# fundamentalvision/BEVFormer

Measured on AMD Instinct MI355X. Metric: BEV-encoder queries/sec (200x200 BEV, 6 cams, 4 lvls), higher is better.
Workload: dtype f32/bf16x3; 1 GPU; bevformer_base BEV encoder forward, 1 frame/step, 200x200 queries, 6 cams, 4 levels, 6 layers, with history BEV; sca_row_order=image, global_batch=1, parallelism=single GPU

## Files before the change

### bevformer_amd/csrc/bevmsda_linear.hip

```cpp
#include "../../include/bevmsda.h"
#include "linear_mfma.h"
#include "linear_pipe.h"
#include "linear_panel.h"
#include "linear_roles.h"
#include "linear_chain.h"
#include "wgrad_mfma.h"
#include "wgrad_tr.h"

namespace {
constexpr bool kLinearPipeDefault = false;
constexpr long long kLinearPipeMaxRows = 8192;
constexpr long long kChainSmallRows = 8192;
inline bool misaligned(const void *p) { return (reinterpret_cast<uintptr_t>(p) & 15u) != 0; }
}

extern "C" {

static int linear_launch(const float *x0, const float *a0, const float *x1, const float *a1, const float *w,
                         const uint16_t *wpack, const float *bias, const bevmsda_linear_desc *d, float *y,
                         void *stream, const int32_t *gidx = nullptr, const float *gscale = nullptr,
                         const float *mask = nullptr, long ldmask = 0, float mask_scale = 1.0f) {
  if (!d) return BEVMSDA_ERR_NULL_POINTER;
  if (d->M < 0 || d->N < 0 || d->K0 < 0 || d->K1 < 0) return BEVMSDA_ERR_BAD_SHAPE;
  if (d->precision != 0 && d->precision != 1) return BEVMSDA_ERR_BAD_OPTION;
// ... 166 lines not shown
  if (nprob < 0 || nprob > bevmsda::kWgMaxProblems || M < 0) return BEVMSDA_ERR_BAD_SHAPE;
  if (precision != 0 && precision != 1) return BEVMSDA_ERR_BAD_OPTION;
  if (nprob == 0 || M == 0) return BEVMSDA_OK;
  if (!probs) return BEVMSDA_ERR_NULL_POINTER;
  if (variant == 2 && workgroups == 0) {
    long long t2 = 0;
    for (int i = 0; i < nprob; ++i) t2 += 1LL * ((probs[i].N + 255) / 256) * ((probs[i].K + 127) / 128);
    const long long s2 = t2 > 0 ? (256 / t2 / 8) * 8 : 0;
    if (s2 < 8 || t2 * s2 < 208) variant = 0;
  }
  bevmsda::WgradMultiArgs a{};
  long long tiles = 0;
  for (int i = 0; i < nprob; ++i) {
    const bevmsda_wgrad_problem &q = probs[i];
    if (q.N <= 0 || q.K <= 0) return BEVMSDA_ERR_BAD_SHAPE;
    if (q.N % 4 != 0 || q.K % 4 != 0 || q.ldg % 4 != 0 || q.ldx % 4 != 0) return BEVMSDA_ERR_UNSUPPORTED;
    if (q.ldg < q.N || q.ldx < q.K || q.ldgw < q.K) return BEVMSDA_ERR_BAD_SHAPE;
    if (!q.g || !q.x || !q.grad_w) return BEVMSDA_ERR_NULL_POINTER;
    if (misaligned(q.g) || misaligned(q.x) || (reinterpret_cast<uintptr_t>(q.grad_w) & 3u) != 0) return BEVMSDA_ERR_MISALIGNED;
    bevmsda::WgradArgs &w = a.p[i];
    w.g = q.g; w.x = q.x; w.ldg = q.ldg; w.ldx = q.ldx; w.gw = q.grad_w; w.ldgw = q.ldgw; w.gb = q.grad_b; w.M = M;
    w.N = q.N; w.K = q.K; w.tiles_n = (q.N + (variant == 2 ? 255 : 127)) / (variant == 2 ? 256 : 128); w.tiles_k = (q.K + 127) / 128;
    a.tile0[i] = static_cast<int>(tiles);
    tiles += 1LL * w.tiles_n * w.tiles_k;
  }
  if (tiles >= (1LL << 20)) return BEVMSDA_ERR_TOO_LARGE;
  a.tile0[nprob] = static_cast<int>(tiles);
  a.nprob = nprob;
  if (workgroups < 0 || workgroups > (1 << 20)) return BEVMSDA_ERR_BAD_OPTION;
  long long slices = workgroups > 0 ? workgroups / tiles : (tiles >= 12 ? (768 + tiles - 1) / tiles : 512 / tiles);
  if (variant == 2 && workgroups == 0) {
    slices = (256 / tiles / 8) * 8;
    if (slices < 8) slices = 8;
  }
  if (slices < 1) slices = 1;
  long long rows = (M + slices - 1) / slices;
  rows = ((rows + 31) / 32) * 32;
  if (rows < 128) rows = 128;
  slices = (M + rows - 1) / rows;
  for (int i = 0; i < nprob; ++i) a.p[i].rows_per_block = static_cast<int>(rows);
  const long long slices8 = ((slices + 7) / 8) * 8;
  if (tiles * slices8 >= (1LL << 31)) return BEVMSDA_ERR_TOO_LARGE;
  const dim3 grid(static_cast<unsigned>(tiles * slices8)), block(256);
  hipStream_t st = static_cast<hipStream_t>(stream);
  if (variant == 2) {
    if (precision == 0) hipLaunchKernelGGL((bevmsda::wgrad_tr2_multi_kernel<3>), grid, dim3(512), 0, st, a);
    else hipLaunchKernelGGL((bevmsda::wgrad_tr2_multi_kernel<1>), grid, dim3(512), 0, st, a);
  } else if (variant == 0) {
    if (precision == 0) hipLaunchKernelGGL((bevmsda::wgrad_tr_multi_kernel<3>), grid, block, 0, st, a);
    else hipLaunchKernelGGL((bevmsda::wgrad_tr_multi_kernel<1>), grid, block, 0, st, a);
  } else {
    if (precision == 0) hipLaunchKernelGGL((bevmsda::wgrad_multi_kernel<3>), grid, block, 0, st, a);
    else hipLaunchKernelGGL((bevmsda::wgrad_multi_kernel<1>), grid, block, 0, st, a);
  }
  return hipGetLastError() == hipSuccess ? BEVMSDA_OK : BEVMSDA_ERR_LAUNCH;
}

int64_t bevmsda_linear_packed_bytes(int N, int K) {
  if (N <= 0 || K <= 0 || K % 32 != 0) return 0;
  return static_cast<int64_t>((N + 127) / 128) * (K / 32) * 2 * 128 * 40 * 2;
}

int bevmsda_linear_pack_weight_f32(const float *w, int64_t ldw, int N, int K, uint16_t *blob, void *stream) {
  if (N <= 0 || K <= 0) return BEVMSDA_ERR_BAD_SHAPE;
  if (K % 32 != 0 || ldw % 4 != 0) return BEVMSDA_ERR_UNSUPPORTED;
  if (ldw < K) return BEVMSDA_ERR_BAD_SHAPE;
  if (!w || !blob) return BEVMSDA_ERR_NULL_POINTER;
  if (misaligned(w) || misaligned(blob)) return BEVMSDA_ERR_MISALIGNED;
  const long long threads = static_cast<long long>((N + 127) / 128) * 128 * (K / 8);
  const long long nb = (threads + 255) / 256;
  if (nb >= (1LL << 31)) return BEVMSDA_ERR_TOO_LARGE;
  hipLaunchKernelGGL(bevmsda::lin_pack_weight_kernel<false>, dim3(static_cast<unsigned>(nb)), dim3(256), 0,
                     static_cast<hipStream_t>(stream), w, static_cast<long>(ldw), N, K, blob);
  return hipGetLastError() == hipSuccess ? BEVMSDA_OK : BEVMSDA_ERR_LAUNCH;
}

int bevmsda_linear_pack_weight_t_f32(const float *wt, int64_t ldwt, int N, int K, uint16_t *blob, void *stream) {
  if (N <= 0 || K <= 0) return BEVMSDA_ERR_BAD_SHAPE;
  if (K % 32 != 0) return BEVMSDA_ERR_UNSUPPORTED;
  if (ldwt < N) return BEVMSDA_ERR_BAD_SHAPE;
  if (!wt || !blob) return BEVMSDA_ERR_NULL_POINTER;
  if (misaligned(blob) || (reinterpret_cast<uintptr_t>(wt) & 3u)) return BEVMSDA_ERR_MISALIGNED;
  const long long threads = static_cast<long long>((N + 127) / 128) * 128 * (K / 8);
  const long long nb = (threads + 255) / 256;
  if (nb >= (1LL << 31)) return BEVMSDA_ERR_TOO_LARGE;
  hipLaunchKernelGGL(bevmsda::lin_pack_weight_kernel<true>, dim3(static_cast<unsigned>(nb)), dim3(256), 0,
                     static_cast<hipStream_t>(stream), wt, static_cast<long>(ldwt), N, K, blob);
  return hipGetLastError() == hipSuccess ? BEVMSDA_OK : BEVMSDA_ERR_LAUNCH;
}

int64_t bevmsda_linear_panel_packed_bytes(int N, int K) {
  if (N <= 0 || K <= 0 || K % bevmsda::kPanelK != 0) return 0;
  return static_cast<int64_t>((N + 63) / 64) * 2 * (K / 16) * 2 * 1024;
}

int bevmsda_linear_panel_pack_weight_f32(const float *w, int64_t ldw, int N, int K, uint16_t *blob, void *stream) {
  if (N <= 0 || K <= 0) return BEVMSDA_ERR_BAD_SHAPE;
  if (K % bevmsda::kPanelK != 0 || ldw % 4 != 0) return BEVMSDA_ERR_UNSUPPORTED;
  if (ldw < K) return BEVMSDA_ERR_BAD_SHAPE;
  if (!w || !blob) return BEVMSDA_ERR_NULL_POINTER;
  if (misaligned(w) || misaligned(blob)) return BEVMSDA_ERR_MISALIGNED;
  const int tiles32 = ((N + 63) / 64) * 2;
  const long long threads = 1LL * tiles32 * (K / 16) * 64;
  const long long nb = (threads + 255) / 256;
  if (nb >= (1LL << 31)) return BEVMSDA_ERR_TOO_LARGE;
  hipLaunchKernelGGL(bevmsda::lin_panel_pack_weight_kernel<false>, dim3(static_cast<unsigned>(nb)), dim3(256), 0,
                     static_cast<hipStream_t>(stream), w, static_cast<long>(ldw), N, K, tiles32, blob);
  return hipGetLastError() == hipSuccess ? BEVMSDA_OK : BEVMSDA_ERR_LAUNCH;
}

int bevmsda_linear_panel_pack_weight_t_f32(const float *wt, int64_t ldwt, int N, int K, uint16_t *blob, void *stream) {
  if (N <= 0 || K <= 0) return BEVMSDA_ERR_BAD_SHAPE;
  if (K % bevmsda::kPanelK != 0) return BEVMSDA_ERR_UNSUPPORTED;
  if (ldwt < N) return BEVMSDA_ERR_BAD_SHAPE;
  if (!wt || !blob) return BEVMSDA_ERR_NULL_POINTER;
  if (misaligned(blob) || (reinterpret_cast<uintptr_t>(wt) & 3u)) return BEVMSDA_ERR_MISALIGNED;
  const int tiles32 = ((N + 63) / 64) * 2;
  const long long threads = 1LL * tiles32 * (K / 16) * 64;
  const long long nb = (threads + 255) / 256;
  if (nb >= (1LL << 31)) return BEVMSDA_ERR_TOO_LARGE;
  hipLaunchKernelGGL(bevmsda::lin_panel_pack_weight_kernel<true>, dim3(static_cast<unsigned>(nb)), dim3(256), 0,
                     static_cast<hipStream_t>(stream), wt, static_cast<long>(ldwt), N, K, tiles32, blob);
  return hipGetLastError() == hipSuccess ? BEVMSDA_OK : BEVMSDA_ERR_LAUNCH;
}

int64_t bevmsda_linear_pack_job_blocks(int N, int K, int kind) {
  if (N <= 0 || K <= 0 || kind < 0 || kind > 3) return 0;
  if (kind & 2) {
    if (K % bevmsda::kPanelK != 0) return 0;
    const long long threads = 1LL * ((N + 63) / 64) * 2 * (K / 16) * 64;
    return (threads + 255) / 256;
  }
  if (K % 32 != 0) return 0;
  const long long threads = static_cast<long long>((N + 127) / 128) * 128 * (K / 8);
  return (threads + 255) / 256;
}

int bevmsda_linear_pack_weights_multi_f32(const bevmsda_pack_job *jobs, int njobs, int64_t blocks, void *stream) {
  static_assert(sizeof(bevmsda_pack_job) == sizeof(bevmsda::PackJob), "bevmsda_pack_job layout");
  if (njobs < 0 || blocks < 0) return BEVMSDA_ERR_BAD_SHAPE;
  if (njobs == 0 || blocks == 0) return BEVMSDA_OK;
  if (!jobs) return BEVMSDA_ERR_NULL_POINTER;
  if (misaligned(jobs)) return BEVMSDA_ERR_MISALIGNED;
  if (blocks >= (1LL << 31)) return BEVMSDA_ERR_TOO_LARGE;
  hipLaunchKernelGGL(bevmsda::lin_pack_weights_multi_kernel, dim3(static_cast<unsigned>(blocks)), dim3(256), 0,
                     static_cast<hipStream_t>(stream), reinterpret_cast<const bevmsda::PackJob *>(jobs), njobs);
  return hipGetLastError() == hipSuccess ? BEVMSDA_OK : BEVMSDA_ERR_LAUNCH;
}

static constexpr int kPanelSkewDefault = 0;
static constexpr long kPanelRolesMinRows = 65536;
static constexpr int kPanelRolesMinCols = 1024;
static constexpr bool kPanelRolesNtStores = true;

static int panel_launch(const float *x0, const float *a0, const float *x1, const float *a1, const int32_t *idx,
                        const float *scale, const uint16_t *wpanel, const float *bias,
                        const bevmsda_linear_desc *d, const bevmsda_layernorm_desc *ln, float *y, void *stream,
                        const int32_t *seg_start, int64_t seg_len, const int64_t *level_shapes, int num_levels,
                        const float *xb = nullptr, int64_t m_split = 0, const int32_t *need = nullptr,
                        int64_t need_rows = 0, int64_t need_len = 0) {
  if (!d) return BEVMSDA_ERR_NULL_POINTER;
  if (d->M < 0 || d->N < 0 || d->K0 < 0 || d->K1 < 0 || d->group_cols < 0) return BEVMSDA_ERR_BAD_SHAPE;
  if (xb && (m_split < 0 || m_split > d->M)) return BEVMSDA_ERR_BAD_SHAPE;
  if (xb && (d->K1 != 0 || a0 || idx || ln || seg_start)) return BEVMSDA_ERR_UNSUPPORTED;
  if (xb && misaligned(xb)) return BEVMSDA_ERR_MISALIGNED;
  if (d->precision != 0 && d->precision != 1) return BEVMSDA_ERR_BAD_OPTION;
  if (d->M == 0 || d->N == 0) return BEVMSDA_OK;
  const int K = d->K0 + d->K1;
  if ((K != 256 && K != 512) || (d->K0 != 256 && d->K0 != 512) || (d->K1 != 0 && d->K1 != 256)) return BEVMSDA_ERR_UNSUPPORTED;
  if (!x0 || !wpanel || !y || (d->K1 > 0 && !x1)) return BEVMSDA_ERR_NULL_POINTER;
  if ((idx == nullptr) != (scale == nullptr)) return BEVMSDA_ERR_NULL_POINTER;
  if (idx && (d->K1 != 0 || a0)) return BEVMSDA_ERR_BAD_SHAPE;
  const int gcols = d->group_cols;
  if (d->N % 4 != 0 || d->ldy % 4 != 0 || d->ldx0 % 4 != 0 || (a0 && d->lda0 % 4 != 0) ||
      (d->K1 > 0 && (d->ldx1 % 4 != 0 || (a1 && d->lda1 % 4 != 0))) || (gcols > 0 && (gcols % 64 != 0 || d->N % gcols != 0)))
    return BEVMSDA_ERR_UNSUPPORTED;
  if (d->ldx0 < d->K0 || d->ldy < (gcols > 0 ? gcols : d->N) || (d->K1 > 0 && d->ldx1 < d->K1)) return BEVMSDA_ERR_BAD_SHAPE;
  if (misaligned(x0) || misaligned(wpanel) || misaligned(y) || (bias && misaligned(bias)) || (a0 && misaligned(a0)) ||
      (d->K1 > 0 && (misaligned(x1) || (a1 && misaligned(a1)))))
    return BEVMSDA_ERR_MISALIGNED;
  const int64_t wbytes = bevmsda_linear_panel_packed_bytes(d->N, K);
  if (wbytes >= (1LL << 31)) return BEVMSDA_ERR_TOO_LARGE;
  if (!ln && 128LL * d->ldy * (d->out_bf16 ? 2 : 4) >= (1LL << 31)) return BEVMSDA_ERR_TOO_LARGE;
  bevmsda::PanelArgs a;
  a.x0 = x0; a.a0 = a0; a.x1 = d->K1 > 0 ? x1 : nullptr; a.a1 = d->K1 > 0 ? a1 : nullptr;
  a.ldx0 = d->ldx0; a.lda0 = d->lda0; a.ldx1 = d->ldx1; a.lda1 = d->lda1;
  a.gidx = idx; a.gscale = scale;
  a.wp = wpanel; a.wp_bytes = static_cast<unsigned>(wbytes);
  a.bias = bias; a.y = y; a.ldy = d->ldy; a.M = d->M; a.N = d->N; a.K0 = d->K0; a.K1 = d->K1;
  a.relu = d->relu ? 1 : 0; a.group_cols = gcols; a.out_bf16 = d->out_bf16 ? 1 : 0;
  a.res = nullptr; a.ldres = 0; a.gamma = a.beta = nullptr; a.eps = 0.f;
  a.xb = xb; a.m_split = m_split;
  a.need = need; a.need_rows = need_rows;
  if (need) {
    if (!xb || d->relu || K != 256) return BEVMSDA_ERR_UNSUPPORTED;
    if (need_rows <= 0 || need_len <= 0) return BEVMSDA_ERR_BAD_SHAPE;
    const int64_t longest = m_split > d->M - m_split ? m_split : d->M - m_split;
    if ((longest + need_rows - 1) / need_rows > need_len) return BEVMSDA_ERR_BAD_SHAPE;
    if ((reinterpret_cast<uintptr_t>(need) & 3u) != 0) return BEVMSDA_ERR_MISALIGNED;
    if (d->reserved[3] != 0) return BEVMSDA_ERR_UNSUPPORTED;
  }
  a.seg_start = seg_start; a.seg_len = seg_len; a.level_shapes = level_shapes; a.num_levels = level_shapes ? num_levels : 0;
  if (seg_start && (seg_len <= 0 || num_levels < 0)) return BEVMSDA_ERR_BAD_SHAPE;
  if (ln) {
    if (d->N != 256 || gcols != 0 || d->relu || d->out_bf16) return BEVMSDA_ERR_UNSUPPORTED;
    if (!ln->gamma || !ln->beta) return BEVMSDA_ERR_NULL_POINTER;
    if (misaligned(ln->gamma) || misaligned(ln->beta) || (ln->res && (misaligned(ln->res) || ln->ldres % 4 != 0 || ln->ldres < d->N)))
      return BEVMSDA_ERR_MISALIGNED;
    a.res = ln->res; a.ldres = ln->ldres; a.gamma = ln->gamma; a.beta = ln->beta; a.eps = ln->eps;
  }
  int shape = d->reserved[2];
  if (shape < 0 || shape > 3) return BEVMSDA_ERR_BAD_OPTION;
  if ((K == 512 || ln) && d->N > 256) return BEVMSDA_ERR_UNSUPPORTED;
  const bool roles_form = !idx && !a.a0 && !a.a1 && !ln && K == 256 && d->N % 32 == 0;
  if (shape == 0 && roles_form && d->N >= kPanelRolesMinCols && d->M >= kPanelRolesMinRows) shape = 3;
  bevmsda_linear_desc d_rule;
  if (shape == 3 && !roles_form) {
    d_rule = *d;
    d_rule.reserved[2] = 0;
    d_rule.reserved[3] = 0;
    d = &d_rule;
    shape = 0;
  }
  if (shape == 3) {
    if (d->reserved[3] < 0 || d->reserved[3] > 4) return BEVMSDA_ERR_BAD_OPTION;
    const int knob = d->reserved[3] == 0 ? (kPanelRolesNtStores ? 2 : 0) : d->reserved[3] & 3;
    const long long nb3 = (d->M + 63) / 64;
    if (nb3 >= (1LL << 31)) return BEVMSDA_ERR_TOO_LARGE;
    a.skew = 0;
    const dim3 g3(static_cast<unsigned>(nb3)), b3(bevmsda::kRolesThreads);
    hipStream_t st3 = static_cast<hipStream_t>(stream);
    if (need) {
      if (d->precision == 0) hipLaunchKernelGGL((bevmsda::linear_roles_kernel<3, kPanelRolesNtStores ? 2 : 0, true, true>), g3, b3, 0, st3, a);
      else hipLaunchKernelGGL((bevmsda::linear_roles_kernel<1, kPanelRolesNtStores ? 2 : 0, true, true>), g3, b3, 0, st3, a);
      return hipGetLastError() == hipSuccess ? BEVMSDA_OK : BEVMSDA_ERR_LAUNCH;
    }
#define BEVMSDA_ROLES(NP_)                                                                                                \
    do {                                                                                                                  \
      switch (knob) {                                                                                                     \
        case 0: hipLaunchKernelGGL((bevmsda::linear_roles_kernel<NP_, 0, true>), g3, b3, 0, st3, a); break;               \
        case 1: hipLaunchKernelGGL((bevmsda::linear_roles_kernel<NP_, 0, false>), g3, b3, 0, st3, a); break;              \
        case 2: hipLaunchKernelGGL((bevmsda::linear_roles_kernel<NP_, 2, true>), g3, b3, 0, st3, a); break;               \
        default: hipLaunchKernelGGL((bevmsda::linear_roles_kernel<NP_, 2, false>), g3, b3, 0, st3, a); break;             \
      }                                                                                                                   \
    } while (0)
    if (d->precision == 0) BEVMSDA_ROLES(3); else BEVMSDA_ROLES(1);
#undef BEVMSDA_ROLES
    return hipGetLastError() == hipSuccess ? BEVMSDA_OK : BEVMSDA_ERR_LAUNCH;
  }
  if (shape == 0) shape = d->N >= 1024 && d->M >= 65536 ? 2 : 1;
  const int bm = shape == 1 ? 64 : 128;
  const long long nb = (d->M + bm - 1) / bm;
  if (nb >= (1LL << 31)) return BEVMSDA_ERR_TOO_LARGE;
  hipStream_t st = static_cast<hipStream_t>(stream);
  const dim3 grid(static_cast<unsigned>(nb));
  int ev = d->reserved[3] >= 32 && d->reserved[3] < 64 ? d->reserved[3] - 32 : -1;
  const bool plain = !idx && !a.a0 && !a.a1 && !ln;
  a.skew = plain && d->reserved[3] == 0 ? kPanelSkewDefault : 0;
  if (d->reserved[3] == 97 || d->reserved[3] == 98) {
  } else if (d->reserved[3] >= 64) {
    if (d->reserved[3] > 98 || !plain) return BEVMSDA_ERR_BAD_OPTION;
    a.skew = d->reserved[3] - 64;
  } else if (ev >= 0) {
    if (ev > 4 || idx || a.a0 || a.a1 || ln) return BEVMSDA_ERR_BAD_OPTION;
  } else if (d->reserved[3] != 0 && d->reserved[3] != 2 && d->reserved[3] != 6) {
    return BEVMSDA_ERR_BAD_OPTION;
  }
  if (need) {
#define BEVMSDA_PANEL_MASKED(NP_)                                                                                              \
    do {                                                                                                                       \
      if (shape == 1) hipLaunchKernelGGL((bevmsda::linear_panel_kernel<NP_, 2, 2, 4, false, 0, 0, 0, false, 2, false, true>), grid, dim3(256), 0, st, a); \
      else hipLaunchKernelGGL((bevmsda::linear_panel_kernel<NP_, 4, 1, 8, false, 0, 0, 0, false, 2, false, true>), grid, dim3(512), 0, st, a);           \
    } while (0)
    if (d->precision == 0) BEVMSDA_PANEL_MASKED(3); else BEVMSDA_PANEL_MASKED(1);
#undef BEVMSDA_PANEL_MASKED
    return hipGetLastError() == hipSuccess ? BEVMSDA_OK : BEVMSDA_ERR_LAUNCH;
  }
  const bool deep = d->reserved[3] == 6;
  if (d->reserved[3] == 97 || d->reserved[3] == 98) {
    if (!plain) return BEVMSDA_ERR_BAD_OPTION;
    const dim3 g128(static_cast<unsigned>((d->M + 127) / 128));
    if (d->precision == 0) {
      if (d->reserved[3] == 97) hipLaunchKernelGGL((bevmsda::linear_panel_kernel<3, 4, 2, 4, false, 0, 0, 0, true, 2>), g128, dim3(256), 0, st, a);
      else hipLaunchKernelGGL((bevmsda::linear_panel_kernel<3, 4, 2, 4, false, 0, 0, 0, true, 4>), g128, dim3(256), 0, st, a);
    } else {
      if (d->reserved[3] == 97) hipLaunchKernelGGL((bevmsda::linear_panel_kernel<1, 4, 2, 4, false, 0, 0, 0, true, 2>), g128, dim3(256), 0, st, a);
      else hipLaunchKernelGGL((bevmsda::linear_panel_kernel<1, 4, 2, 4, false, 0, 0, 0, true, 4>), g128, dim3(256), 0, st, a);
    }
    return hipGetLastError() == hipSuccess ? BEVMSDA_OK : BEVMSDA_ERR_LAUNCH;
  }
  if (ev > 0) {
#define BEVMSDA_PANEL_EV(NP_)                                                                                                  \
    do {                                                                                                                       \
      if (shape == 1) {                                                                                                        \
        if (ev == 1) hipLaunchKernelGGL((bevmsda::linear_panel_kernel<NP_, 2, 2, 4, false, 0, 0, 0, true, 2>), grid, dim3(256), 0, st, a);  \
        else if (ev == 2) hipLaunchKernelGGL((bevmsda::linear_panel_kernel<NP_, 2, 2, 4, false, 0, 0, 0, false, 4>), grid, dim3(256), 0, st, a); \
        else if (ev == 3) hipLaunchKernelGGL((bevmsda::linear_panel_kernel<NP_, 2, 2, 4, false, 0, 0, 0, true, 4>), grid, dim3(256), 0, st, a);  \
        else hipLaunchKernelGGL((bevmsda::linear_panel_kernel<NP_, 2, 2, 4, false, 0, 0, 0, false, 2, true>), grid, dim3(256), 0, st, a);    \
      } else {                                                                                                                 \
        if (ev == 1) hipLaunchKernelGGL((bevmsda::linear_panel_kernel<NP_, 4, 1, 8, false, 0, 0, 0, true, 2>), grid, dim3(512), 0, st, a);  \
        else if (ev == 2) hipLaunchKernelGGL((bevmsda::linear_panel_kernel<NP_, 4, 1, 8, false, 0, 0, 0, false, 4>), grid, dim3(512), 0, st, a); \
        else if (ev == 3) hipLaunchKernelGGL((bevmsda::linear_panel_kernel<NP_, 4, 1, 8, false, 0, 0, 0, true, 4>), grid, dim3(512), 0, st, a);  \
        else hipLaunchKernelGGL((bevmsda::linear_panel_kernel<NP_, 4, 1, 8, false, 0, 0, 0, false, 2, true>), grid, dim3(512), 0, st, a);    \
      }                                                                                                                        \
    } while (0)
    if (d->precision == 0) BEVMSDA_PANEL_EV(3); else BEVMSDA_PANEL_EV(1);
#undef BEVMSDA_PANEL_EV
    return hipGetLastError() == hipSuccess ? BEVMSDA_OK : BEVMSDA_ERR_LAUNCH;
  }
#define BEVMSDA_PANEL2(NP_, LN_, PRE_)                                                                                   \
  do {                                                                                                                   \
    if (shape == 1 && deep && (PRE_) == 0)                                                                               \
      hipLaunchKernelGGL((bevmsda::linear_panel_kernel<NP_, 2, 2, 4, LN_, PRE_, 0, 0, false, 6>), grid, dim3(256), 0, st, a); \
    else if (shape == 1) hipLaunchKernelGGL((bevmsda::linear_panel_kernel<NP_, 2, 2, 4, LN_, PRE_>), grid, dim3(256), 0, st, a); \
    else hipLaunchKernelGGL((bevmsda::linear_panel_kernel<NP_, 4, 1, 8, LN_, PRE_>), grid, dim3(512), 0, st, a);           \
  } while (0)
#define BEVMSDA_PANEL(NP_, LN_)                              \
  do {                                                       \
    if (idx) BEVMSDA_PANEL2(NP_, LN_, 2);                    \
    else if (a.a0 || a.a1) BEVMSDA_PANEL2(NP_, LN_, 1);      \
    else BEVMSDA_PANEL2(NP_, LN_, 0);                        \
  } while (0)
  if (d->precision == 0) { if (ln) BEVMSDA_PANEL(3, true); else BEVMSDA_PANEL(3, false); }
  else { if (ln) BEVMSDA_PANEL(1, true); else BEVMSDA_PANEL(1, false); }
#undef BEVMSDA_PANEL2
#undef BEVMSDA_PANEL
  return hipGetLastError() == hipSuccess ? BEVMSDA_OK : BEVMSDA_ERR_LAUNCH;
}

int bevmsda_linear_panel_f32(const float *x0, const float *a0, const float *x1, const float *a1, const int32_t *idx,
                             const float *scale, const uint16_t *wpanel, const float *bias,
                             const bevmsda_linear_desc *d, const bevmsda_layernorm_desc *ln, float *y, void *stream) {
  return panel_launch(x0, a0, x1, a1, idx, scale, wpanel, bias, d, ln, y, stream, nullptr, 0, nullptr, 0);
}

int bevmsda_linear_panel_segments_f32(const float *x0, const uint16_t *wpanel, const float *bias, const bevmsda_linear_desc *d,
                                      const int32_t *seg_start, int64_t seg_len, const int64_t *level_shapes,
                                      int num_levels, float *y, void *stream) {
  if (!seg_start) return BEVMSDA_ERR_NULL_POINTER;
  return panel_launch(x0, nullptr, nullptr, nullptr, nullptr, nullptr, wpanel, bias, d, nullptr, y, stream, seg_start, seg_len,
                      level_shapes, num_levels);
}

int bevmsda_linear_panel_rows2_f32(const float *x_lo, const float *x_hi, int64_t m_split, const uint16_t *wpanel, const float *bias,
                                   const bevmsda_linear_desc *d, float *y, void *stream) {
  if (!x_hi) return BEVMSDA_ERR_NULL_POINTER;
  return panel_launch(x_lo, nullptr, nullptr, nullptr, nullptr, nullptr, wpanel, bias, d, nullptr, y, stream, nullptr, 0, nullptr, 0,
                      x_hi, m_split);
}

int bevmsda_linear_panel_rows2_masked_f32(const float *x_lo, const float *x_hi, int64_t m_split, const uint16_t *wpanel,
                                          const float *bias, const bevmsda_linear_desc *d, const int32_t *need, int64_t need_rows,
                                          int64_t need_len, float *y, void *stream) {
  if (!x_hi || !need) return BEVMSDA_ERR_NULL_POINTER;
  return panel_launch(x_lo, nullptr, nullptr, nullptr, nullptr, nullptr, wpanel, bias, d, nullptr, y, stream, nullptr, 0, nullptr, 0,
                      x_hi, m_split, need, need_rows, need_len);
}

struct ChainTail {
  const float *first; long long ld_first;
  const float *pos; long long ld_pos;
  const uint16_t *w3p; const float *b3;
  float *proj; long long ld_proj;
  int n3;
};

static int ffn_chain_launch(const float *rows, const int32_t *idx, const float *scale, const uint16_t *w0p, const float *b0,
                            const float *res, const float *gamma0, const float *beta0, const uint16_t *w1p, const float *b1,
                            const uint16_t *w2p, const float *b2, const float *gamma1, const float *beta1,
                            const bevmsda_chain_desc *d, float *y, void *stream, bool save, float *sv_z0, float *sv_x,
                            float *sv_h, float *sv_z1, const float *dk0 = nullptr, const float *dkh = nullptr,
                            const float *dk1 = nullptr, const ChainTail *tp = nullptr) {
  if (!d) return BEVMSDA_ERR_NULL_POINTER;
  const bool drop = dk0 || dkh || dk1;
  if (tp) {
    if (save || drop) return BEVMSDA_ERR_BAD_OPTION;
    if (tp->n3 <= 0 || tp->n3 > 256 || tp->n3 % 64 != 0) return BEVMSDA_ERR_UNSUPPORTED;
    if (d->M > 0 && (!tp->first || !tp->w3p || !tp->proj)) return BEVMSDA_ERR_NULL_POINTER;
    if (tp->ld_first % 4 != 0 || tp->ld_proj % 4 != 0 || (tp->pos && tp->ld_pos % 4 != 0)) return BEVMSDA_ERR_UNSUPPORTED;
    if (tp->ld_first < 256 || tp->ld_proj < tp->n3 || (tp->pos && tp->ld_pos < 256)) return BEVMSDA_ERR_BAD_SHAPE;
    if (misaligned(tp->first) || misaligned(tp->w3p) || misaligned(tp->proj) || (tp->pos && misaligned(tp->pos)) ||
        (tp->b3 && misaligned(tp->b3)))
      return BEVMSDA_ERR_MISALIGNED;
  }
// ... 288 lines not shown
```

### bevformer_amd/csrc/linear_roles.h

```cpp
#pragma once
#include "linear_panel.h"

namespace bevmsda {

constexpr int kRolesMfmaWaves = 8;
constexpr int kRolesStoreWaves = 4;
constexpr int kRolesThreads = (kRolesMfmaWaves + kRolesStoreWaves) * 64;

__device__ __forceinline__ int roles_flag_load(int *p) {
  return __builtin_amdgcn_readfirstlane(__hip_atomic_load(p, __ATOMIC_RELAXED, __HIP_MEMORY_SCOPE_WORKGROUP));
}
__device__ __forceinline__ void roles_flag_set(int *p, int v) {
  __hip_atomic_store(p, v, __ATOMIC_RELAXED, __HIP_MEMORY_SCOPE_WORKGROUP);
}

template <int NPROD, int STAUX, bool PRIO, bool MASKED = false>
__global__ void __launch_bounds__(kRolesThreads) linear_roles_kernel(const PanelArgs a) {
  static_assert(NPROD == 1 || NPROD == 3, "NPROD");
  constexpr bool LO = NPROD == 3;
  constexpr int NPL = LO ? 2 : 1;
  constexpr int MT = 2;
  constexpr int NW = kRolesMfmaWaves;
  constexpr int BM = MT * 32;
  constexpr int NPAIR = (BM / 8) * 4;
// ... 76 lines not shown
      lin_split8<LO>(va, vb, hi, lo);
      *reinterpret_cast<uint4 *>(slot) = hi;
      if (LO) *reinterpret_cast<uint4 *>(slot + 1024) = lo;
    }
  } else if (wave == NW && lane < 2 * NW) {
    flags[lane] = 0;
  }
  __syncthreads();
  if (wave >= NW) {
    const int w0 = wave - NW, w1 = w0 + 4;
    const int n0 = w0 < nct ? (nct - w0 + NW - 1) / NW : 0;
    const int n1 = w1 < nct ? (nct - w1 + NW - 1) / NW : 0;
    const int rr = lane >> 3, c = lane & 7;
    const int es = a.out_bf16 ? 2 : 4;
    const unsigned ldy_b = static_cast<unsigned>(a.ldy) * es;
    auto drain = [&](int w, int t) {
      const unsigned char *sl = slots + w * SLOT_BYTES + rr * 128 + ((c ^ rr) << 4);
      float4 v[8];
#pragma unroll
      for (int p = 0; p < 8; ++p) v[p] = *reinterpret_cast<const float4 *>(sl + p * 1024);
      asm volatile("s_waitcnt lgkmcnt(0)" ::: "memory");
      roles_flag_set(&flags[NW + w], t + 1);
      const int ct = w + t * NW;
      const int n0c = ct * 32;
      const int grp = a.group_cols > 0 ? n0c / a.group_cols : 0;
      const int soff_e = n0c - grp * a.group_cols;
      const long firstel = (static_cast<long>(grp) * a.M + m0) * a.ldy;
      unsigned char *base = reinterpret_cast<unsigned char *>(a.y) + firstel * es;
      const __amdgpu_buffer_rsrc_t yr = __builtin_amdgcn_make_buffer_rsrc(base, 0, static_cast<int>(rows_here * ldy_b), 0x00020000);
      if (a.out_bf16) {
#pragma unroll
        for (int p = 0; p < 8; ++p) {
          const panel_u32x2 d = {lin_pack2(v[p].x, v[p].y), lin_pack2(v[p].z, v[p].w)};
          __builtin_amdgcn_raw_buffer_store_b64(d, yr, static_cast<int>((p * 8 + rr) * ldy_b) + c * 8, soff_e * 2, STAUX);
        }
      } else {
#pragma unroll
        for (int p = 0; p < 8; ++p) {
          const panel_u32x4 d = {__float_as_uint(v[p].x), __float_as_uint(v[p].y), __float_as_uint(v[p].z), __float_as_uint(v[p].w)};
          __builtin_amdgcn_raw_buffer_store_b128(d, yr, static_cast<int>((p * 8 + rr) * ldy_b) + c * 16, soff_e * 4, STAUX);
        }
      }
    };
    int d0 = 0, d1 = 0;
    while (d0 < n0 || d1 < n1) {
      bool did = false;
      if (d0 < n0 && roles_flag_load(&flags[w0]) > d0) { drain(w0, d0); ++d0; did = true; }
      if (d1 < n1 && roles_flag_load(&flags[w1]) > d1) { drain(w1, d1); ++d1; did = true; }
      if (!did) __builtin_amdgcn_s_sleep(1);
    }
    return;
  }

  if constexpr (PRIO) __builtin_amdgcn_s_setprio(1);

  unsigned f_addr[4];
  unsigned c_off[MT][4];
  {
    int ll = lane;
    asm volatile("" : "+v"(ll));
    const int r_ = ll & 31, h_ = ll >> 5;
    const int q0_ = ((r_ >> 2) & 1) | ((r_ >> 4) << 1);
    const int rl_ = ((r_ & 3) << 1) | ((r_ >> 3) & 1);
#pragma unroll
    for (int sc = 0; sc < 4; ++sc) f_addr[sc] = static_cast<unsigned>(q0_ * 4 * 2048 + (rl_ * 8 + (((2 * sc + h_) ^ (r_ & 7)))) * 16);
#pragma unroll
    for (int i = 0; i < MT; ++i)
#pragma unroll
      for (int g = 0; g < 4; ++g) {
        const int r = i * 32 + r_, cc = 2 * g + h_;
        c_off[i][g] = static_cast<unsigned>(wave * SLOT_BYTES + r * 128 + ((cc ^ (r & 7)) << 4));
      }
  }
  float4 bfr[4];
  int t = 0;
  for (int ct = wave; ct < nct; ct += NW, ++t) {
    const int ct_next = ct + NW;
    lin_bf16x8 af[2][MT][NPL];
    auto aload = [&](int set, int s) {
      const unsigned base = f_addr[s & 3] + (s >> 2) * 2048;
#pragma unroll
      for (int i = 0; i < MT; ++i)
#pragma unroll
        for (int pl = 0; pl < NPL; ++pl)
          af[set][i][pl] = *reinterpret_cast<const lin_bf16x8 *>(lds + base + i * (4 * 4 * 2048) + pl * 1024);
    };
    aload(0, 0);
    if (a.bias != nullptr) {
#pragma unroll
      for (int g = 0; g < 4; ++g) bfr[g] = *reinterpret_cast<const float4 *>(a.bias + ct * 32 + 4 * (lane >> 5) + 8 * g);
    }
#pragma unroll
    for (int s = 0; s < 16; ++s) {
      if (s + WD < 16) {
        wload((s + WD) % RS, ct, s + WD);
      } else if (ct_next < nct) {
        wload((s + WD) % RS, ct_next, s + WD - 16);
      }
      if (s + 1 < 16) aload((s + 1) & 1, s + 1);
      __builtin_amdgcn_sched_barrier(0);
#pragma unroll
      for (int i = 0; i < MT; ++i) {
        if (LO) {
          acc[i] = __builtin_amdgcn_mfma_f32_32x32x16_bf16(wf[s % RS][0], af[s & 1][i][1], acc[i], 0, 0, 0);
          acc[i] = __builtin_amdgcn_mfma_f32_32x32x16_bf16(wf[s % RS][1], af[s & 1][i][0], acc[i], 0, 0, 0);
        }
        acc[i] = __builtin_amdgcn_mfma_f32_32x32x16_bf16(wf[s % RS][0], af[s & 1][i][0], acc[i], 0, 0, 0);
      }
      __builtin_amdgcn_sched_barrier(0);
    }
    if (ct_next < nct && (16 % RS) != 0) {
      lin_bf16x8 tmp[WD][NPL];
#pragma unroll
      for (int k = 0; k < WD; ++k)
#pragma unroll
        for (int pl = 0; pl < NPL; ++pl) tmp[k][pl] = wf[(16 + k) % RS][pl];
#pragma unroll
      for (int k = 0; k < WD; ++k)
#pragma unroll
        for (int pl = 0; pl < NPL; ++pl) wf[k][pl] = tmp[k][pl];
    }
    if (a.bias != nullptr) {
#pragma unroll
      for (int i = 0; i < MT; ++i)
#pragma unroll
        for (int g = 0; g < 4; ++g) {
          acc[i][4 * g] += bfr[g].x; acc[i][4 * g + 1] += bfr[g].y;
          acc[i][4 * g + 2] += bfr[g].z; acc[i][4 * g + 3] += bfr[g].w;
        }
    }
    if (a.relu) {
#pragma unroll
      for (int i = 0; i < MT; ++i)
#pragma unroll
        for (int r = 0; r < 16; ++r) acc[i][r] = acc[i][r] < 0.f ? 0.f : acc[i][r];
    }
    while (roles_flag_load(&flags[NW + wave]) < t) __builtin_amdgcn_s_sleep(1);
    asm volatile("" ::: "memory");
#pragma unroll
    for (int i = 0; i < MT; ++i)
#pragma unroll
      for (int g = 0; g < 4; ++g)
        *reinterpret_cast<float4 *>(slots + c_off[i][g]) =
            make_float4(acc[i][4 * g], acc[i][4 * g + 1], acc[i][4 * g + 2], acc[i][4 * g + 3]);
    asm volatile("s_waitcnt lgkmcnt(0)" ::: "memory");
    roles_flag_set(&flags[wave], t + 1);
#pragma unroll
    for (int i = 0; i < MT; ++i)
#pragma unroll
      for (int r = 0; r < 16; ++r) acc[i][r] = 0.f;
  }
}

}
```

### bevformer_amd/modes.py

```python
import contextlib
import copy
import os
import threading

import torch

GEMM_MODES = ("split", "bf16", "native")
GEMM_KERNELS = (None, "first", "first64", "pipe", "panel", "panel64", "panel128", "panel64w2", "panel64w6") + tuple(
    f"panel{bm}e{v}" for bm in (64, 128) for v in (1, 2, 3, 4)) + tuple(
    f"panel{bm}s{n}" for bm in (64, 128) for n in (0, 1, 2, 3, 4, 6, 8, 12)) + ("panel128d2", "panel128d4") + (
    "panelr", "panelr1", "panelr2", "panelr3", "panelr4")


class Modes:
    __slots__ = ("value_storage", "fused", "fused_train", "gemm", "gemm_variant", "gemm_pack", "train_forward_mfma",
                 "gemm_kernel", "ln_fuse", "wgrad", "bf16_lanes8", "fused_wpe", "fused_lds_pad_kb", "chain_shape", "grad_thread", "train_chain", "wgrad_workgroups", "wgrad_variant", "stack_free", "weight_views", "flatten_params", "fused_save", "chain_backward", "grad_arena", "overlap_value_proj", "use_grad_arena", "fused_spec", "fused_capacity_launch", "graph_repack", "tsa_seam", "chain_gather_all", "plan_on_side", "tile_halo")

    def __init__(self):
        env = os.environ.get
        self.value_storage = torch.float32
        self.fused = True
        self.fused_train = env("BEVMSDA_FUSED_TRAIN", "1") == "1"
        self.gemm = env("BEVMSDA_GEMM", "split")
        self.gemm_variant = int(env("BEVMSDA_GEMM_VARIANT")) if env("BEVMSDA_GEMM_VARIANT") else None
        self.gemm_pack = env("BEVMSDA_GEMM_PACK", "1") == "1"
        self.train_forward_mfma = env("BEVMSDA_TRAIN_FWD_MFMA", "1") == "1"
        k = env("BEVMSDA_GEMM_KERNEL", "")
        self.gemm_kernel = k if k in GEMM_KERNELS[1:] else None
        self.ln_fuse = env("BEVMSDA_FUSE_LN", "1") == "1"
        self.wgrad = env("BEVMSDA_WGRAD", "1") == "1"
        self.bf16_lanes8 = env("BEVMSDA_BF16_LANES8") is not None
        self.fused_wpe = int(env("BEVMSDA_FUSED_WPE", "0"))
        self.fused_spec = int(env("BEVMSDA_FUSED_SPEC", "0"))
        self.fused_capacity_launch = {"0": False, "1": True}.get(env("BEVMSDA_FUSED_CAPACITY", "auto"), "auto")
        self.graph_repack = env("BEVMSDA_GRAPH_REPACK", "0") == "1"
        self.fused_lds_pad_kb = int(env("BEVMSDA_FUSED_LDS_PAD", "0"))
        self.stack_free = env("BEVMSDA_STACK_FREE", "1") == "1"
        self.weight_views = env("BEVMSDA_WEIGHT_VIEWS", "1") == "1"
        self.flatten_params = env("BEVMSDA_FLATTEN_PARAMS", "1") == "1"
        self.fused_save = int(env("BEVMSDA_FUSED_SAVE", "1"))
        self.chain_backward = env("BEVMSDA_CHAIN_BWD", "1") == "1"
        self.chain_shape = int(env("BEVMSDA_CHAIN_SHAPE", "0"))
        self.grad_thread = env("BEVMSDA_GRAD_THREAD", "1") == "1"
        self.train_chain = env("BEVMSDA_TRAIN_CHAIN", "1") == "1"
        self.wgrad_workgroups = int(env("BEVMSDA_WGRAD_WGS", "0"))
        self.wgrad_variant = int(env("BEVMSDA_WGRAD_VARIANT", "2"))
        self.grad_arena = None
        self.use_grad_arena = env("BEVMSDA_GRAD_ARENA", "1") == "1"
        self.tsa_seam = env("BEVMSDA_TSA_SEAM", "1") == "1"
        self.tile_halo = max(0, int(env("BEVMSDA_TILE_HALO", "0") or 0))
        self.chain_gather_all = env("BEVMSDA_CHAIN_GATHER_ALL", "1") == "1"
        self.plan_on_side = env("BEVMSDA_PLAN_SIDE", "1") == "1"
        self.overlap_value_proj = env("BEVMSDA_OVERLAP", "1") == "1"
        assert self.gemm in GEMM_MODES, f"BEVMSDA_GEMM must be one of {GEMM_MODES}"

    def snapshot(self):
        return copy.copy(self)


_PROCESS = Modes()
_TLS = threading.local()


def process_defaults():
    return _PROCESS


def current():
    stack = getattr(_TLS, "stack", None)
    return stack[-1] if stack else _PROCESS


@contextlib.contextmanager
def activate(modes):
    stack = getattr(_TLS, "stack", None)
    if stack is None:
        stack = _TLS.stack = []
    stack.append(modes)
    try:
        yield modes
    finally:
        stack.pop()


@contextlib.contextmanager
def using(**overrides):
    m = current().snapshot()
    for k, v in overrides.items():
        if k not in Modes.__slots__:
            raise AttributeError(f"unknown mode {k!r}")
        setattr(m, k, v)
    with activate(m):
        yield m
```

Measured before the change: 10.52 million BEV queries/s.

## Add persistent roles GEMM kernel with cross-panel producer/consumer pipelining

After: 10.43 million BEV queries/s. About the same (-0.9%).

```diff
diff --git a/bevformer_amd/csrc/bevmsda_linear.hip b/bevformer_amd/csrc/bevmsda_linear.hip
--- a/bevformer_amd/csrc/bevmsda_linear.hip
+++ b/bevformer_amd/csrc/bevmsda_linear.hip
@@ -342,6 +342,19 @@
 static constexpr long kPanelRolesMinRows = 65536;
 static constexpr int kPanelRolesMinCols = 1024;
 static constexpr bool kPanelRolesNtStores = true;
+static constexpr bool kPanelRolesPersistent = true;
+
+static int device_cu_count() {
+  constexpr int kMaxDevices = 64;
+  static int cached[kMaxDevices] = {};
+  int dev = 0;
+  if (hipGetDevice(&dev) != hipSuccess || dev < 0) return 0;
+  if (dev < kMaxDevices && cached[dev] > 0) return cached[dev];
+  int n = 0;
+  if (hipDeviceGetAttribute(&n, hipDeviceAttributeMultiprocessorCount, dev) != hipSuccess || n <= 0) return 0;
+  if (dev < kMaxDevices) cached[dev] = n;
+  return n;
+}
 
 static int panel_launch(const float *x0, const float *a0, const float *x1, const float *a1, const int32_t *idx,
                         const float *scale, const uint16_t *wpanel, const float *bias,
@@ -413,13 +426,31 @@
     shape = 0;
   }
   if (shape == 3) {
-    if (d->reserved[3] < 0 || d->reserved[3] > 4) return BEVMSDA_ERR_BAD_OPTION;
-    const int knob = d->reserved[3] == 0 ? (kPanelRolesNtStores ? 2 : 0) : d->reserved[3] & 3;
+    if (d->reserved[3] < 0 || d->reserved[3] > 6) return BEVMSDA_ERR_BAD_OPTION;
+    const bool persistent = d->reserved[3] == 6 || (d->reserved[3] == 0 && kPanelRolesPersistent);
+    const int knob = d->reserved[3] == 0 || d->reserved[3] >= 5 ? (kPanelRolesNtStores ? 2 : 0) : d->reserved[3] & 3;
     const long long nb3 = (d->M + 63) / 64;
     if (nb3 >= (1LL << 31)) return BEVMSDA_ERR_TOO_LARGE;
     a.skew = 0;
-    const dim3 g3(static_cast<unsigned>(nb3)), b3(bevmsda::kRolesThreads);
+    const dim3 b3(bevmsda::kRolesThreads);
     hipStream_t st3 = static_cast<hipStream_t>(stream);
+    if (persistent) {
+      const int cus = device_cu_count();
+      if (cus <= 0) return BEVMSDA_ERR_LAUNCH;
+      const long long per64 = (nb3 + 63) / 64;
+      const long long wgs = nb3 < cus ? nb3 : (per64 > cus ? per64 : cus);
+      const dim3 gp(static_cast<unsigned>(wgs));
+      constexpr int kSt = kPanelRolesNtStores ? 2 : 0;
+      if (need) {
+        if (d->precision == 0) hipLaunchKernelGGL((bevmsda::linear_roles_persistent_kernel<3, kSt, true, true>), gp, b3, 0, st3, a);
+        else hipLaunchKernelGGL((bevmsda::linear_roles_persistent_kernel<1, kSt, true, true>), gp, b3, 0, st3, a);
+      } else {
+        if (d->precision == 0) hipLaunchKernelGGL((bevmsda::linear_roles_persistent_kernel<3, kSt, true>), gp, b3, 0, st3, a);
+        else hipLaunchKernelGGL((bevmsda::linear_roles_persistent_kernel<1, kSt, true>), gp, b3, 0, st3, a);
+      }
+      return hipGetLastError() == hipSuccess ? BEVMSDA_OK : BEVMSDA_ERR_LAUNCH;
+    }
+    const dim3 g3(static_cast<unsigned>(nb3));
     if (need) {
       if (d->precision == 0) hipLaunchKernelGGL((bevmsda::linear_roles_kernel<3, kPanelRolesNtStores ? 2 : 0, true, true>), g3, b3, 0, st3, a);
       else hipLaunchKernelGGL((bevmsda::linear_roles_kernel<1, kPanelRolesNtStores ? 2 : 0, true, true>), g3, b3, 0, st3, a);
diff --git a/bevformer_amd/csrc/linear_roles.h b/bevformer_amd/csrc/linear_roles.h
--- a/bevformer_amd/csrc/linear_roles.h
+++ b/bevformer_amd/csrc/linear_roles.h
@@ -252,4 +252,310 @@
   }
 }
 
+
+constexpr int kRolesFlagFull = 0, kRolesFlagFree = 8, kRolesFlagDone = 16, kRolesFlagReady = 24, kRolesFlagWords = 32;
+
+template <int N>
+__device__ __forceinline__ bool roles_flags_reached(int *base, int lane, int v) {
+  const int x = __hip_atomic_load(base + (lane & (N - 1)), __ATOMIC_RELAXED, __HIP_MEMORY_SCOPE_WORKGROUP);
+  return __builtin_amdgcn_ballot_w64(x < v) == 0;
 }
+
+template <int NPROD, int STAUX, bool PRIO, bool MASKED = false>
+__global__ void __launch_bounds__(kRolesThreads) linear_roles_persistent_kernel(const PanelArgs a) {
+  static_assert(NPROD == 1 || NPROD == 3, "NPROD");
+  constexpr bool LO = NPROD == 3;
+  constexpr int NPL = LO ? 2 : 1;
+  constexpr int MT = 2;
+  constexpr int NW = kRolesMfmaWaves;
+  constexpr int BM = MT * 32;
+  constexpr int NPAIR = (BM / 8) * 4;
+  constexpr int PANEL_BYTES = NPAIR * 2048;
+  constexpr int SLOT_BYTES = BM * 32 * 4;
+  constexpr int WD = 2, RS = WD + 1;
+  static_assert(NW == 2 * kRolesStoreWaves, "two row blocks and two C slots per store wavefront");
+  __shared__ __attribute__((aligned(16))) unsigned char lds[PANEL_BYTES + NW * SLOT_BYTES];
+  __shared__ int flags[kRolesFlagWords];
+
+  const int tid = threadIdx.x;
+  const int lane = tid & 63;
+  const int wave = __builtin_amdgcn_readfirstlane(tid >> 6);
+  const int npanel = static_cast<int>((a.M + BM - 1) / BM);
+  const int stride = static_cast<int>(gridDim.x);
+  long halo = 0;
+  if (a.seg_start != nullptr) {
+    for (int l = 0; l < a.num_levels; ++l) halo = a.level_shapes[2 * l + 1] > halo ? a.level_shapes[2 * l + 1] : halo;
+    halo += a.num_levels > 0 ? 1 : 0;
+  }
+  const int npos_all = (npanel - static_cast<int>(blockIdx.x) + stride - 1) / stride;
+  const int npos = npos_all < 64 ? npos_all : 64;
+  auto panel_of = [&](int j) { return static_cast<int>(blockIdx.x) + j * stride; };
+  auto pos_used = [&](int j) {
+    const long m0 = static_cast<long>(panel_of(j)) * BM;
+    int used = 1;
+    if (a.seg_start != nullptr) {
+      const long first = m0 - halo > 0 ? m0 - halo : 0;
+      const long last = (m0 + BM + halo < a.M ? m0 + BM + halo : a.M) - 1;
+      const int s_lo = static_cast<int>(first / a.seg_len), s_hi = static_cast<int>(last / a.seg_len);
+      used = 0;
+      for (int sg = s_lo; sg <= s_hi; ++sg) used |= a.seg_start[sg + 1] - a.seg_start[sg];
+    }
+    if constexpr (MASKED) {
+      if (used != 0 && !panel_rows_needed(a, m0, BM)) used = 0;
+    }
+    return used != 0;
+  };
+  unsigned long long used_mask;
+  if (a.seg_start == nullptr && !MASKED) {
+    used_mask = npos >= 64 ? ~0ULL : (1ULL << npos) - 1ULL;
+  } else {
+    used_mask = __builtin_amdgcn_ballot_w64(lane < npos && pos_used(lane));
+    __builtin_amdgcn_s_waitcnt(0x0F70);
+  }
+  auto next_pos = [&](int j) {
+    const unsigned long long m = j < 64 ? used_mask >> j : 0ULL;
+    return m != 0 ? j + static_cast<int>(__builtin_ctzll(m)) : npos;
+  };
+  if (tid < kRolesFlagWords) flags[tid] = 0;
+  __syncthreads();
+  const int j_first = next_pos(0);
+  const int nct = a.N / 32;
+  const int nstep = kPanelK / 16;
+  unsigned char *slots = lds + PANEL_BYTES;
+
+  if (wave >= NW) {
+    const int sw = wave - NW;
+    const int w0 = sw, w1 = sw + 4;
+    const int n0 = w0 < nct ? (nct - w0 + NW - 1) / NW : 0;
+    const int n1 = w1 < nct ? (nct - w1 + NW - 1) / NW : 0;
+    const int rr = lane >> 3, c = lane & 7;
+    const int es = a.out_bf16 ? 2 : 4;
+    const unsigned ldy_b = static_cast<unsigned>(a.ldy) * es;
+    float4 nx[16];
+    auto stage = [&](int j) {
+      const long m0 = static_cast<long>(panel_of(j)) * BM;
+#pragma unroll
+      for (int u = 0; u < 2; ++u) {
+        const int row = panel_row_of(2 * sw + u, rr);
+        long gm = m0 + row;
+        if (gm >= a.M) gm = a.M - 1;
+        const bool second_block = a.xb != nullptr && gm >= a.m_split;
+        const float *src = (second_block ? a.xb + (gm - a.m_split) * a.ldx0 : a.x0 + gm * a.ldx0) + (c ^ (row & 7)) * 4;
+#pragma unroll
+        for (int pp = 0; pp < 4; ++pp) {
+          nx[(u * 4 + pp) * 2] = *reinterpret_cast<const float4 *>(src + pp * 64);
+          nx[(u * 4 + pp) * 2 + 1] = *reinterpret_cast<const float4 *>(src + pp * 64 + 32);
+        }
+      }
+      asm volatile("" ::: "memory");
+    };
+    auto plant = [&]() {
+#pragma unroll
+      for (int u = 0; u < 2; ++u)
+#pragma unroll
+        for (int pp = 0; pp < 4; ++pp) {
+          unsigned char *slot = lds + ((2 * sw + u) * 4 + pp) * 2048 + lane * 16;
+          uint4 hi, lo;
+          lin_split8<LO>(nx[(u * 4 + pp) * 2], nx[(u * 4 + pp) * 2 + 1], hi, lo);
+          *reinterpret_cast<uint4 *>(slot) = hi;
+          if (LO) *reinterpret_cast<uint4 *>(slot + 1024) = lo;
+        }
+    };
+    auto drain = [&](int w, int g, int j, int t) {
+      const unsigned char *sl = slots + w * SLOT_BYTES + rr * 128 + ((c ^ rr) << 4);
+      float4 v[8];
+#pragma unroll
+      for (int q = 0; q < 8; ++q) v[q] = *reinterpret_cast<const float4 *>(sl + q * 1024);
+      asm volatile("s_waitcnt lgkmcnt(0)" ::: "memory");
+      roles_flag_set(&flags[kRolesFlagFree + w], g + 1);
+      const long m0 = static_cast<long>(panel_of(j)) * BM;
+      const long rows_here = a.M - m0 < BM ? a.M - m0 : BM;
+      const int ct = w + t * NW;
+      const int n0c = ct * 32;
+      const int grp = a.group_cols > 0 ? n0c / a.group_cols : 0;
+      const int soff_e = n0c - grp * a.group_cols;
+      const long firstel = (static_cast<long>(grp) * a.M + m0) * a.ldy;
+      unsigned char *base = reinterpret_cast<unsigned char *>(a.y) + firstel * es;
+      const __amdgpu_buffer_rsrc_t yr = __builtin_amdgcn_make_buffer_rsrc(base, 0, static_cast<int>(rows_here * ldy_b), 0x00020000);
+      if (a.out_bf16) {
+#pragma unroll
+        for (int q = 0; q < 8; ++q) {
+          const panel_u32x2 d = {lin_pack2(v[q].x, v[q].y), lin_pack2(v[q].z, v[q].w)};
+          __builtin_amdgcn_raw_buffer_store_b64(d, yr, static_cast<int>((q * 8 + rr) * ldy_b) + c * 8, soff_e * 2, STAUX);
+        }
+      } else {
+#pragma unroll
+        for (int q = 0; q < 8; ++q) {
+          const panel_u32x4 d = {__float_as_uint(v[q].x), __float_as_uint(v[q].y), __float_as_uint(v[q].z), __float_as_uint(v[q].w)};
+          __builtin_amdgcn_raw_buffer_store_b128(d, yr, static_cast<int>((q * 8 + rr) * ldy_b) + c * 16, soff_e * 4, STAUX);
+        }
+      }
+    };
+    int wp = j_first, wk = 0;
+    int p0 = j_first, p1 = j_first;
+    int t0 = 0, t1 = 0, g0 = 0, g1 = 0;
+    if (n0 == 0) p0 = npos;
+    if (n1 == 0) p1 = npos;
+    if (wp < npos) stage(wp);
+    while (wp < npos || p0 < npos || p1 < npos) {
+      bool did = false;
+      if (wp < npos && roles_flags_reached<NW>(&flags[kRolesFlagDone], lane, wk)) {
+        asm volatile("" ::: "memory");
+        plant();
+        asm volatile("s_waitcnt lgkmcnt(0)" ::: "memory");
+        roles_flag_set(&flags[kRolesFlagReady + sw], ++wk);
+        wp = next_pos(wp + 1);
+        if (wp < npos) stage(wp);
+        did = true;
+      }
+      if (p0 < npos && roles_flag_load(&flags[kRolesFlagFull + w0]) > g0) {
+        drain(w0, g0, p0, t0);
+        ++g0;
+        if (++t0 == n0) { t0 = 0; p0 = next_pos(p0 + 1); }
+        did = true;
+      }
+      if (p1 < npos && roles_flag_load(&flags[kRolesFlagFull + w1]) > g1) {
+        drain(w1, g1, p1, t1);
+        ++g1;
+        if (++t1 == n1) { t1 = 0; p1 = next_pos(p1 + 1); }
+        did = true;
+      }
+      if (!did) __builtin_amdgcn_s_sleep(1);
+    }
+    return;
+  }
+
+  __amdgpu_buffer_rsrc_t wrsrc = __builtin_amdgcn_make_buffer_rsrc(const_cast<uint16_t *>(a.wp), 0,
+                                                                   static_cast<int>(a.wp_bytes), 0x00020000);
+  const int wlane = lane * 16;
+  lin_f32x16 acc[MT];
+  lin_bf16x8 wf[RS][NPL];
+  auto wload = [&](int st, int ct, int sg) {
+#pragma unroll
+    for (int pl = 0; pl < NPL; ++pl) {
+      const int so = ((ct * nstep + sg) * 2 + pl) * 1024;
+      wf[st][pl] = __builtin_bit_cast(lin_bf16x8, __builtin_amdgcn_raw_buffer_load_b128(wrsrc, wlane, so, 0));
+    }
+  };
+  if (wave >= nct || j_first >= npos) {
+    int k = 0;
+    for (int j = j_first; j < npos; j = next_pos(j + 1)) roles_flag_set(&flags[kRolesFlagDone + wave], ++k);
+    return;
+  }
+  if constexpr (PRIO) __builtin_amdgcn_s_setprio(1);
+  unsigned f_addr[4];
+  unsigned c_off[MT][4];
+  {
+    int ll = lane;
+    asm volatile("" : "+v"(ll));
+    const int r_ = ll & 31, h_ = ll >> 5;
+    const int q0_ = ((r_ >> 2) & 1) | ((r_ >> 4) << 1);
+    const int rl_ = ((r_ & 3) << 1) | ((r_ >> 3) & 1);
+#pragma unroll
+    for (int sc = 0; sc < 4; ++sc) f_addr[sc] = static_cast<unsigned>(q0_ * 4 * 2048 + (rl_ * 8 + (((2 * sc + h_) ^ (r_ & 7)))) * 16);
+#pragma unroll
+    for (int i = 0; i < MT; ++i)
+#pragma unroll
+      for (int g = 0; g < 4; ++g) {
+        const int r = i * 32 + r_, cc = 2 * g + h_;
+        c_off[i][g] = static_cast<unsigned>(wave * SLOT_BYTES + r * 128 + ((cc ^ (r & 7)) << 4));
+      }
+  }
+#pragma unroll
+  for (int i = 0; i < MT; ++i)
+#pragma unroll
+    for (int r = 0; r < 16; ++r) acc[i][r] = 0.f;
+#pragma unroll
+  for (int k = 0; k < WD; ++k) wload(k, wave, k);
+  float4 bfr[4];
+  int t = 0;
+  int k = 0;
+  for (int j = j_first; j < npos; j = next_pos(j + 1), ++k) {
+    while (!roles_flags_reached<kRolesStoreWaves>(&flags[kRolesFlagReady], lane, k + 1)) __builtin_amdgcn_s_sleep(1);
+    asm volatile("" ::: "memory");
+    for (int ct = wave; ct < nct; ct += NW, ++t) {
+      const bool last_ct = ct + NW >= nct;
+      const int ct_next = last_ct ? wave : ct + NW;
+      lin_bf16x8 af[2][MT][NPL];
+      auto aload = [&](int set, int s) {
+        const unsigned base = f_addr[s & 3] + (s >> 2) * 2048;
+#pragma unroll
+        for (int i = 0; i < MT; ++i)
+#pragma unroll
+          for (int pl = 0; pl < NPL; ++pl)
+            af[set][i][pl] = *reinterpret_cast<const lin_bf16x8 *>(lds + base + i * (4 * 4 * 2048) + pl * 1024);
+      };
+      aload(0, 0);
+      if (a.bias != nullptr) {
+#pragma unroll
+        for (int g = 0; g < 4; ++g) bfr[g] = *reinterpret_cast<const float4 *>(a.bias + ct * 32 + 4 * (lane >> 5) + 8 * g);
+      }
+#pragma unroll
+      for (int s = 0; s < 16; ++s) {
+        if (s + WD < 16) wload((s + WD) % RS, ct, s + WD);
+        else wload((s + WD) % RS, ct_next, s + WD - 16);
+        if (s + 1 < 16) aload((s + 1) & 1, s + 1);
+        __builtin_amdgcn_sched_barrier(0);
+#pragma unroll
+        for (int i = 0; i < MT; ++i) {
+          if (LO) {
+            acc[i] = __builtin_amdgcn_mfma_f32_32x32x16_bf16(wf[s % RS][0], af[s & 1][i][1], acc[i], 0, 0, 0);
+            acc[i] = __builtin_amdgcn_mfma_f32_32x32x16_bf16(wf[s % RS][1], af[s & 1][i][0], acc[i], 0, 0, 0);
+          }
+          acc[i] = __builtin_amdgcn_mfma_f32_32x32x16_bf16(wf[s % RS][0], af[s & 1][i][0], acc[i], 0, 0, 0);
+        }
+        __builtin_amdgcn_sched_barrier(0);
+      }
+      if ((16 % RS) != 0) {
+        lin_bf16x8 tmp[WD][NPL];
+#pragma unroll
+        for (int j = 0; j < WD; ++j)
+#pragma unroll
+          for (int pl = 0; pl < NPL; ++pl) tmp[j][pl] = wf[(16 + j) % RS][pl];
+#pragma unroll
+        for (int j = 0; j < WD; ++j)
+#pragma unroll
+          for (int pl = 0; pl < NPL; ++pl) wf[j][pl] = tmp[j][pl];
+      }
+      if (last_ct) {
+        asm volatile("s_waitcnt lgkmcnt(0)" ::: "memory");
+        roles_flag_set(&flags[kRolesFlagDone + wave], k + 1);
+      }
+      if (a.bias != nullptr) {
+#pragma unroll
+        for (int i = 0; i < MT; ++i)
+#pragma unroll
+          for (int g = 0; g < 4; ++g) {
+            acc[i][4 * g] += bfr[g].x; acc[i][4 * g + 1] += bfr[g].y;
+            acc[i][4 * g + 2] += bfr[g].z; acc[i][4 * g + 3] += bfr[g].w;
+          }
+      }
+      if (a.relu) {
+#pragma unroll
+        for (int i = 0; i < MT; ++i)
+#pragma unroll
+          for (int r = 0; r < 16; ++r) acc[i][r] = acc[i][r] < 0.f ? 0.f : acc[i][r];
+      }
+      while (roles_flag_load(&flags[kRolesFlagFree + wave]) < t) __builtin_amdgcn_s_sleep(1);
+      asm volatile("" ::: "memory");
+#pragma unroll
+      for (int i = 0; i < MT; ++i)
+#pragma unroll
+        for (int g = 0; g < 4; ++g)
+          *reinterpret_cast<float4 *>(slots + c_off[i][g]) =
+              make_float4(acc[i][4 * g], acc[i][4 * g + 1], acc[i][4 * g + 2], acc[i][4 * g + 3]);
+      asm volatile("s_waitcnt lgkmcnt(0)" ::: "memory");
+      roles_flag_set(&flags[kRolesFlagFull + wave], t + 1);
+#pragma unroll
+      for (int i = 0; i < MT; ++i)
+#pragma unroll
+        for (int r = 0; r < 16; ++r) acc[i][r] = 0.f;
+    }
+  }
+#pragma unroll
+  for (int j = 0; j < WD; ++j)
+#pragma unroll
+    for (int pl = 0; pl < NPL; ++pl) asm volatile("" ::"v"(wf[j][pl]));
+}
+
+}
diff --git a/bevformer_amd/modes.py b/bevformer_amd/modes.py
--- a/bevformer_amd/modes.py
+++ b/bevformer_amd/modes.py
@@ -9,7 +9,7 @@
 GEMM_KERNELS = (None, "first", "first64", "pipe", "panel", "panel64", "panel128", "panel64w2", "panel64w6") + tuple(
     f"panel{bm}e{v}" for bm in (64, 128) for v in (1, 2, 3, 4)) + tuple(
     f"panel{bm}s{n}" for bm in (64, 128) for n in (0, 1, 2, 3, 4, 6, 8, 12)) + ("panel128d2", "panel128d4") + (
-    "panelr", "panelr1", "panelr2", "panelr3", "panelr4")
+    "panelr", "panelr1", "panelr2", "panelr3", "panelr4", "panelr5", "panelr6")
 
 
 class Modes:
```
